# ipastore/glue-factory-colon

Measured on AMD Instinct MI355X. Metric: image-pairs/sec (SuperPoint+LightGlue, 1024 kpts, 640x480), higher is better.
Workload: dtype f32; 1 GPU; SuperPoint-open + LightGlue, 1024 kpts, 640x480 synthetic pairs (BASELINE.json configs[1]); keypoints=1024, parallelism=dp1 (pairs sharded, one final gather), weights=name-seeded seed 0 (no network), pairs_gathered=32, rccl_ranks=1

## Files before the change

### glue-factory-colon_amd/csrc/gemm.hip

```cpp
#include <stdlib.h>

#include "common.h"

#define GBK 32

struct GemmArgs {
  const float* A0;
  const float* A1;
  const float* W;
  const float* bias;
  const float* scale;
  const float* shift;
  const float* residual;
  const float* rot_cos;
  const float* rot_sin;
  const float* rot_cs;
  float* Y;
  long long strideA, strideW, strideY;
  int lda0, lda1, ldw, ldy;
  int K0, K1, M, N, rot_cols;
  float alpha;
  int xcd_remap;
#if defined(GEMM_DIAG) && (GEMM_DIAG & 16)
  unsigned long long* stamps;
#endif
};
#if defined(GEMM_DIAG) && (GEMM_DIAG & 16)
static unsigned long long* g_diag_stamps = nullptr;
extern "C" void gfc_diag_set_gemm_stamps(void* p) { g_diag_stamps = (unsigned long long*)p; }
#define GEMM_STAMP(i_)                                                                               \
  do {                                                                                               \
    if (g.stamps && lane == 0) stamp_base[i_] = __builtin_readcyclecounter();                        \
  } while (0)
#else
#define GEMM_STAMP(i_) do {} while (0)
#endif

template <int MODE, int NS, int RPS, int ELD>
__device__ __forceinline__ void gemm_epilogue_round_fast(const GemmArgs& g, const float* patch, float* Y, int row0, int er,
                                                         int ec, int colb, int rd, float4 bi4, float4 sc4, float4 sh4) {
  float4 opa = make_float4(0.f, 0.f, 0.f, 0.f), opb = opa;
  const float* pa = nullptr;
  const float* pb = nullptr;
  size_t pstep = (size_t)RPS * 64;
  if constexpr (MODE == 1) {
    pa = g.rot_cos + (size_t)row0 * 64 + rd;
    pb = g.rot_sin + (size_t)row0 * 64 + rd;
    opa = *reinterpret_cast<const float4*>(pa);
    opb = *reinterpret_cast<const float4*>(pb);
  } else if constexpr (MODE == 2) {
    pa = g.residual + (size_t)row0 * g.ldy + colb;
    pstep = (size_t)RPS * g.ldy;
    opa = *reinterpret_cast<const float4*>(pa);
  } else if constexpr (MODE == 3) {
    pa = g.rot_cs + (size_t)row0 * 64 + rd;
    opa = *reinterpret_cast<const float4*>(pa);
  }
  float* yp = Y + (size_t)row0 * g.ldy + colb;
  const size_t ystep = (size_t)RPS * g.ldy;
#pragma unroll
  for (int i = 0; i < NS; ++i) {
    float4 na = opa, nb = opb;
    if (i + 1 < NS) {
      if constexpr (MODE != 0) {
        pa += pstep;
        na = *reinterpret_cast<const float4*>(pa);
      }
      if constexpr (MODE == 1) {
        pb += pstep;
        nb = *reinterpret_cast<const float4*>(pb);
      }
    }
    float4 v = *reinterpret_cast<const float4*>(patch + (er + RPS * i) * ELD + ec);
    v.x += bi4.x; v.y += bi4.y; v.z += bi4.z; v.w += bi4.w;
    if constexpr (MODE == 1) {
      const float x = v.x, y = v.y, zz = v.z, w = v.w;
      v.x = x * opa.x + (-y) * opb.x;
      v.y = y * opa.y + x * opb.y;
      v.z = zz * opa.z + (-w) * opb.z;
      v.w = w * opa.w + zz * opb.w;
    }
    if constexpr (MODE == 3) {
      const float x = v.x, y = v.y, zz = v.z, w = v.w;
      v.x = x * opa.x + (-y) * opa.y;
      v.y = y * opa.x + x * opa.y;
      v.z = zz * opa.z + (-w) * opa.w;
      v.w = w * opa.z + zz * opa.w;
    }
    v.x = v.x * sc4.x + sh4.x; v.y = v.y * sc4.y + sh4.y; v.z = v.z * sc4.z + sh4.z; v.w = v.w * sc4.w + sh4.w;
    v.x *= g.alpha; v.y *= g.alpha; v.z *= g.alpha; v.w *= g.alpha;
    if constexpr (MODE == 2) { v.x = opa.x + v.x; v.y = opa.y + v.y; v.z = opa.z + v.z; v.w = opa.w + v.w; }
    *reinterpret_cast<float4*>(yp) = v;
    yp += ystep;
    opa = na; opb = nb;
  }
}

template <int NW, int MT, int MTN = MT>
__device__ __forceinline__ void gemm_epilogue(const GemmArgs& g, f32x16 (&acc)[MT][MTN], float* smem, float* Y, int m0,
                                              int n0, int wm, int wn, int lane, int wave) {
  constexpr int WT = 32 * MTN;
  constexpr int WTM = 32 * MT;
  const int l31 = lane & 31, h = lane >> 5;
  if (((g.rot_cos == nullptr && g.rot_cs == nullptr) || n0 >= g.rot_cols) && g.residual == nullptr) {
#pragma unroll
    for (int nt = 0; nt < MTN; ++nt) {
      const int col = n0 + wn * WT + nt * 32 + l31;
      const bool col_ok = col < g.N;
      const int cc = col_ok ? col : g.N - 1;
      float bi = g.bias ? g.bias[cc] : 0.f;
      float sc = g.scale ? g.scale[cc] : 1.f;
      float sh = g.shift ? g.shift[cc] : 0.f;
      asm volatile("" : "+v"(bi), "+v"(sc), "+v"(sh));
      const bool full = m0 + wm * WTM + MT * 32 <= g.M && n0 + wn * WT + MTN * 32 <= g.N;
#pragma unroll
      for (int mt = 0; mt < MT; ++mt) {
        const int row0 = m0 + wm * WTM + mt * 32;
        if (full) {
          float* yp = Y + (size_t)(row0 + 4 * h) * g.ldy + col;
#pragma unroll
          for (int r = 0; r < 16; ++r) {
            const float v = ((acc[mt][nt][r] + bi) * sc + sh) * g.alpha;
            yp[(size_t)((r & 3) + 8 * (r >> 2)) * g.ldy] = v;
          }
        } else {
#pragma unroll
          for (int r = 0; r < 16; ++r) {
            const int row = row0 + acc_row(r, h);
            const float v = ((acc[mt][nt][r] + bi) * sc + sh) * g.alpha;
            if (row < g.M && col_ok) Y[(size_t)row * g.ldy + col] = v;
          }
        }
      }
    }
    return;
  }
  constexpr int ELD = WT + 4;
  constexpr int LPR = WT / 4;
  constexpr int RPS = 64 / LPR;
  float* patch = smem + wave * 32 * ELD;
  const bool vec_ok = (g.ldy % 4 == 0) && ((reinterpret_cast<size_t>(Y) & 15) == 0) &&
                      (!g.residual || (reinterpret_cast<size_t>(g.residual) & 15) == 0);
  const int er = lane / LPR, ec = (lane % LPR) * 4;
  const int colb = n0 + wn * WT + ec;
  float4 bi4 = make_float4(0.f, 0.f, 0.f, 0.f), sc4 = make_float4(1.f, 1.f, 1.f, 1.f), sh4 = bi4;
  {
    float* bp4 = reinterpret_cast<float*>(&bi4);
    float* sp4 = reinterpret_cast<float*>(&sc4);
    float* hp4 = reinterpret_cast<float*>(&sh4);
#pragma unroll
    for (int j = 0; j < 4; ++j) {
      const int cc = min(colb + j, g.N - 1);
      if (g.bias) bp4[j] = g.bias[cc];
      if (g.scale) { sp4[j] = g.scale[cc]; hp4[j] = g.shift[cc]; }
    }
  }
  const bool rot = (g.rot_cos != nullptr || g.rot_cs != nullptr) && colb < g.rot_cols;
  const int rd = colb & 63;
  asm volatile("" : "+v"(bi4.x), "+v"(bi4.y), "+v"(bi4.z), "+v"(bi4.w));
  asm volatile("" : "+v"(sc4.x), "+v"(sc4.y), "+v"(sc4.z), "+v"(sc4.w));
  asm volatile("" : "+v"(sh4.x), "+v"(sh4.y), "+v"(sh4.z), "+v"(sh4.w));
  const bool rot_w = (g.rot_cos != nullptr || g.rot_cs != nullptr) && n0 + wn * WT < g.rot_cols;
  const bool fast = vec_ok && m0 + wm * WTM + MT * 32 <= g.M && n0 + wn * WT + WT <= g.N && !(rot_w && g.residual);
#pragma unroll
  for (int mt = 0; mt < MT; ++mt) {
    if (fast) {
      constexpr int NS = 32 / RPS;
      const int row0 = m0 + wm * WTM + mt * 32 + er;
      __builtin_amdgcn_fence(__ATOMIC_RELEASE, "wavefront");
      __builtin_amdgcn_wave_barrier();
#pragma unroll
      for (int nt = 0; nt < MTN; ++nt)
#pragma unroll
        for (int r = 0; r < 16; ++r) patch[acc_row(r, h) * ELD + nt * 32 + l31] = acc[mt][nt][r];
      __builtin_amdgcn_fence(__ATOMIC_ACQ_REL, "wavefront");
      __builtin_amdgcn_wave_barrier();
      if (rot_w && g.rot_cs) gemm_epilogue_round_fast<3, NS, RPS, ELD>(g, patch, Y, row0, er, ec, colb, rd, bi4, sc4, sh4);
      else if (rot_w) gemm_epilogue_round_fast<1, NS, RPS, ELD>(g, patch, Y, row0, er, ec, colb, rd, bi4, sc4, sh4);
      else if (g.residual) gemm_epilogue_round_fast<2, NS, RPS, ELD>(g, patch, Y, row0, er, ec, colb, rd, bi4, sc4, sh4);
      else gemm_epilogue_round_fast<0, NS, RPS, ELD>(g, patch, Y, row0, er, ec, colb, rd, bi4, sc4, sh4);
      continue;
    }
    __builtin_amdgcn_fence(__ATOMIC_RELEASE, "wavefront");
    __builtin_amdgcn_wave_barrier();
#pragma unroll
    for (int nt = 0; nt < MTN; ++nt)
#pragma unroll
      for (int r = 0; r < 16; ++r) patch[acc_row(r, h) * ELD + nt * 32 + l31] = acc[mt][nt][r];
    __builtin_amdgcn_fence(__ATOMIC_ACQ_REL, "wavefront");
    __builtin_amdgcn_wave_barrier();
#pragma unroll
    for (int i = 0; i < 32 / RPS; ++i) {
      const int lr = er + RPS * i;
      const int row = m0 + wm * WTM + mt * 32 + lr;
      float4 v = *reinterpret_cast<const float4*>(patch + lr * ELD + ec);
      if (row >= g.M) continue;
      v.x += bi4.x; v.y += bi4.y; v.z += bi4.z; v.w += bi4.w;
      if (rot) {
        float4 c, sn;
        if (g.rot_cs) {
          const float4 cs = *reinterpret_cast<const float4*>(g.rot_cs + (size_t)row * 64 + rd);
          c = make_float4(cs.x, cs.x, cs.z, cs.z);
          sn = make_float4(cs.y, cs.y, cs.w, cs.w);
        } else {
          c = *reinterpret_cast<const float4*>(g.rot_cos + (size_t)row * 64 + rd);
          sn = *reinterpret_cast<const float4*>(g.rot_sin + (size_t)row * 64 + rd);
        }
        const float x = v.x, y = v.y, zz = v.z, w = v.w;
        v.x = x * c.x + (-y) * sn.x;
        v.y = y * c.y + x * sn.y;
        v.z = zz * c.z + (-w) * sn.z;
        v.w = w * c.w + zz * sn.w;
      }
      v.x = v.x * sc4.x + sh4.x; v.y = v.y * sc4.y + sh4.y; v.z = v.z * sc4.z + sh4.z; v.w = v.w * sc4.w + sh4.w;
      v.x *= g.alpha; v.y *= g.alpha; v.z *= g.alpha; v.w *= g.alpha;
      const size_t o = (size_t)row * g.ldy + colb;
      if (vec_ok && colb + 3 < g.N) {
        if (g.residual) {
          const float4 rs = *reinterpret_cast<const float4*>(g.residual + o);
          v.x = rs.x + v.x; v.y = rs.y + v.y; v.z = rs.z + v.z; v.w = rs.w + v.w;
        }
        *reinterpret_cast<float4*>(Y + o) = v;
      } else {
        const float* vp = reinterpret_cast<const float*>(&v);
#pragma unroll
        for (int j = 0; j < 4; ++j)
          if (colb + j < g.N) Y[o + j] = g.residual ? g.residual[o + j] + vp[j] : vp[j];
      }
    }
  }
}

template <int NW, int MT, int BK, int MTN = MT>
__global__ __launch_bounds__(128 * NW, MT * MTN > 4 ? 2 : (BK == 16 ? 4 : 2)) void gemm_nt_kernel(GemmArgs g) {
  constexpr int T = 128 * NW;
  constexpr int GBM = 64 * MT;
  constexpr int BN = 32 * MTN * NW;
  constexpr int GLD = BK + 4;
  constexpr int C4 = BK / 4;
  constexpr int RPP = T / C4;
  constexpr int NA = GBM / RPP;
  constexpr int NB = BN / RPP;
  constexpr int TILE = (GBM + BN) * GLD;
  extern __shared__ __attribute__((aligned(16))) float smem[];

  const int tid = threadIdx.x;
  const int lane = tid & 63, wave = tid >> 6;
  const int l31 = lane & 31, h = lane >> 5;
  const int wm = wave / NW, wn = wave % NW;
  unsigned bx = blockIdx.x, by = blockIdx.y, bz = blockIdx.z;
  if (g.xcd_remap) {
    const unsigned per_z = gridDim.x * gridDim.y;
    unsigned t = gfc_xcd_chunk(bx + gridDim.x * (by + gridDim.y * bz), per_z * gridDim.z);
    bz = t / per_z;
    t -= bz * per_z;
    by = t / gridDim.x;
    bx = t - by * gridDim.x;
  }
  const int m0 = by * GBM, n0 = bx * BN;
  const long long z = bz;
  const float* A0 = g.A0 + z * g.strideA;
  const float* A1 = g.A1 ? g.A1 + z * g.strideA : nullptr;
  const float* W = g.W + z * g.strideW;
  float* Y = g.Y + z * g.strideY;
  const int ktiles = (g.K0 + g.K1) / BK;
#if defined(GEMM_DIAG) && (GEMM_DIAG & 16)
  unsigned long long* stamp_base =
      g.stamps ? g.stamps + ((size_t)(blockIdx.x + gridDim.x * (blockIdx.y + gridDim.y * blockIdx.z)) * (T / 64) + wave) * 8
               : nullptr;
  if (g.stamps && lane == 0) {
    unsigned hw, xcc;
    asm volatile("s_getreg_b32 %0, hwreg(HW_REG_HW_ID)" : "=s"(hw));
    asm volatile("s_getreg_b32 %0, hwreg(HW_REG_XCC_ID)" : "=s"(xcc));
    stamp_base[5] = hw;
    stamp_base[6] = xcc;
  }
  GEMM_STAMP(0);
#endif

  const int s_c4 = (tid % C4) * 4;
  const int q_ = tid / C4;
  const int s_r0 = C4 == 4 ? ((q_ & ~7) | ((q_ & 1) << 2) | ((q_ >> 1) & 3)) : q_;
  const int ar0 = min(m0 + s_r0, g.M - 1), ar1 = min(m0 + s_r0 + RPP, g.M - 1);
  const int ar2 = min(m0 + s_r0 + 2 * RPP, g.M - 1), ar3 = min(m0 + s_r0 + 3 * RPP, g.M - 1);
  const float* w0p = W + (size_t)min(n0 + s_r0, g.N - 1) * g.ldw + s_c4;
  const float* w1p = W + (size_t)min(n0 + s_r0 + RPP, g.N - 1) * g.ldw + s_c4;
  const float* w2p = W + (size_t)min(n0 + s_r0 + 2 * RPP, g.N - 1) * g.ldw + s_c4;
  const float* w3p = W + (size_t)min(n0 + s_r0 + 3 * RPP, g.N - 1) * g.ldw + s_c4;
  static_assert((NB == 1 || NB == 2 || NB == 4) && (NA == 1 || NA == 2 || NA == 4), "staging layout");
  float4 areg0, areg1, areg2, areg3, wreg0, wreg1, wreg2, wreg3;
  areg1 = wreg1 = areg2 = areg3 = wreg2 = wreg3 = make_float4(0.f, 0.f, 0.f, 0.f);
#define GEMM_LOAD_TILE(kt)                                                                           \
  do {                                                                                               \
    const int k0_ = (kt) * BK;                                                                       \
    const bool first_ = k0_ < g.K0;                                                                  \
    const float* ab_ = (first_ ? A0 : A1) + (first_ ? k0_ : k0_ - g.K0) + s_c4;                      \
    const size_t ld_ = first_ ? g.lda0 : g.lda1;                                                     \
    areg0 = *reinterpret_cast<const float4*>(ab_ + ar0 * ld_);                                       \
    if constexpr (NA >= 2) areg1 = *reinterpret_cast<const float4*>(ab_ + ar1 * ld_);                \
    if constexpr (NA == 4) {                                                                         \
      areg2 = *reinterpret_cast<const float4*>(ab_ + ar2 * ld_);                                     \
      areg3 = *reinterpret_cast<const float4*>(ab_ + ar3 * ld_);                                     \
    }                                                                                                \
    wreg0 = *reinterpret_cast<const float4*>(w0p + k0_);                                             \
    if constexpr (NB >= 2) wreg1 = *reinterpret_cast<const float4*>(w1p + k0_);                      \
    if constexpr (NB == 4) {                                                                         \
      wreg2 = *reinterpret_cast<const float4*>(w2p + k0_);                                           \
      wreg3 = *reinterpret_cast<const float4*>(w3p + k0_);                                           \
    }                                                                                                \
  } while (0)
#define GEMM_STORE_TILE(buf_)                                                                        \
  do {                                                                                               \
    float* as_ = smem + (buf_) * TILE + s_r0 * GLD + s_c4;                                           \
    float* bs_ = as_ + GBM * GLD;                                                                    \
    *reinterpret_cast<float4*>(as_) = areg0;                                                         \
    if constexpr (NA >= 2) *reinterpret_cast<float4*>(as_ + RPP * GLD) = areg1;                      \
    if constexpr (NA == 4) {                                                                         \
      *reinterpret_cast<float4*>(as_ + 2 * RPP * GLD) = areg2;                                       \
      *reinterpret_cast<float4*>(as_ + 3 * RPP * GLD) = areg3;                                       \
    }                                                                                                \
    *reinterpret_cast<float4*>(bs_) = wreg0;                                                         \
    if constexpr (NB >= 2) *reinterpret_cast<float4*>(bs_ + RPP * GLD) = wreg1;                      \
    if constexpr (NB == 4) {                                                                         \
      *reinterpret_cast<float4*>(bs_ + 2 * RPP * GLD) = wreg2;                                       \
      *reinterpret_cast<float4*>(bs_ + 3 * RPP * GLD) = wreg3;                                       \
    }                                                                                                \
  } while (0)

  f32x16 acc[MT][MTN];
#pragma unroll
  for (int mt = 0; mt < MT; ++mt)
#pragma unroll
    for (int nt = 0; nt < MTN; ++nt)
#pragma unroll
      for (int r = 0; r < 16; ++r) acc[mt][nt][r] = 0.f;

  const int a_off = (wm * 32 * MT + l31) * GLD + 4 * h;
  const int b_off = GBM * GLD + (wn * 32 * MTN + l31) * GLD + 4 * h;

  GEMM_LOAD_TILE(0);
  GEMM_STORE_TILE(0);
  if (ktiles > 1) GEMM_LOAD_TILE(1);
  __syncthreads();
  GEMM_STAMP(1);
  for (int kt = 0; kt < ktiles; ++kt) {
    if (kt + 1 < ktiles) {
      GEMM_STORE_TILE((kt + 1) & 1);
      if (kt + 2 < ktiles) GEMM_LOAD_TILE(kt + 2);
    }
    const float* ap = smem + (kt & 1) * TILE + a_off;
    const float* bp = smem + (kt & 1) * TILE + b_off;
#pragma unroll
    for (int gk = 0; gk < BK / 8; ++gk) {
      float4 af[MT], bf[MTN];
#pragma unroll
      for (int mt = 0; mt < MT; ++mt) af[mt] = *reinterpret_cast<const float4*>(ap + mt * 32 * GLD + 8 * gk);
#pragma unroll
      for (int nt = 0; nt < MTN; ++nt) bf[nt] = *reinterpret_cast<const float4*>(bp + nt * 32 * GLD + 8 * gk);
#pragma unroll
      for (int mt = 0; mt < MT; ++mt)
#pragma unroll
        for (int nt = 0; nt < MTN; ++nt) {
          acc[mt][nt] = mfma32(af[mt].x, bf[nt].x, acc[mt][nt]);
          acc[mt][nt] = mfma32(af[mt].y, bf[nt].y, acc[mt][nt]);
          acc[mt][nt] = mfma32(af[mt].z, bf[nt].z, acc[mt][nt]);
          acc[mt][nt] = mfma32(af[mt].w, bf[nt].w, acc[mt][nt]);
        }
    }
    __syncthreads();
  }
  GEMM_STAMP(2);

  gemm_epilogue<NW, MT, MTN>(g, acc, smem, Y, m0, n0, wm, wn, lane, wave);
#if defined(GEMM_DIAG) && (GEMM_DIAG & 16)
  GEMM_STAMP(3);
  asm volatile("s_waitcnt vmcnt(0)" ::: "memory");
  GEMM_STAMP(4);
#endif
}

#define GW_BN 512

__device__ __forceinline__ float halfwave_transpose_sum32(const float (&x)[32], int l31) {
  float y16[16], y8[8], y4[4], y2[2];
  const bool b0 = l31 & 1, b1 = l31 & 2, b2 = l31 & 4, b3 = l31 & 8, b4 = l31 & 16;
#pragma unroll
  for (int i = 0; i < 16; ++i) {
    const float mine = b0 ? x[16 + i] : x[i], theirs = b0 ? x[i] : x[16 + i];
    y16[i] = mine + __shfl_xor(theirs, 1);
  }
#pragma unroll
  for (int i = 0; i < 8; ++i) {
    const float mine = b1 ? y16[8 + i] : y16[i], theirs = b1 ? y16[i] : y16[8 + i];
    y8[i] = mine + __shfl_xor(theirs, 2);
  }
#pragma unroll
  for (int i = 0; i < 4; ++i) {
    const float mine = b2 ? y8[4 + i] : y8[i], theirs = b2 ? y8[i] : y8[4 + i];
    y4[i] = mine + __shfl_xor(theirs, 4);
  }
#pragma unroll
  for (int i = 0; i < 2; ++i) {
    const float mine = b3 ? y4[2 + i] : y4[i], theirs = b3 ? y4[i] : y4[2 + i];
    y2[i] = mine + __shfl_xor(theirs, 8);
  }
  const float mine = b4 ? y2[1] : y2[0], theirs = b4 ? y2[0] : y2[1];
  return mine + __shfl_xor(theirs, 16);
}

#define FF_HLD 148
template <bool MLP>
__global__ __launch_bounds__(512, 2) void gemm_rows512_ln_gelu_kernel(GemmArgs g, const float* __restrict__ gamma,
                                                                      const float* __restrict__ beta,
                                                                      const float* __restrict__ W3, int ldw3,
                                                                      const float* __restrict__ b3) {
  constexpr int BM = 128, BK = 16, LD = BK + 4, C4 = BK / 4;
  constexpr int TILE = (BM + GW_BN) * LD;
  extern __shared__ __attribute__((aligned(16))) float smem[];
  const int tid = threadIdx.x, lane = tid & 63, wave = tid >> 6;
  const int l31 = lane & 31, h = lane >> 5;
  const int wm = wave >> 2, wn = wave & 3;
  const int m0 = blockIdx.x * BM;
  const float* A0 = g.A0;
  const float* A1 = g.A1;
  const int ktiles = (g.K0 + g.K1) / BK;
#if defined(GEMM_DIAG) && (GEMM_DIAG & 16)
  unsigned long long* stamp_base = g.stamps ? g.stamps + ((size_t)blockIdx.x * 8 + wave) * 8 : nullptr;
  if (g.stamps && lane == 0) {
    unsigned hw, xcc;
    asm volatile("s_getreg_b32 %0, hwreg(HW_REG_HW_ID)" : "=s"(hw));
    asm volatile("s_getreg_b32 %0, hwreg(HW_REG_XCC_ID)" : "=s"(xcc));
    stamp_base[5] = hw;
    stamp_base[6] = xcc;
  }
  GEMM_STAMP(0);
#endif

  const int s_c4 = (tid % C4) * 4;
  const int q_ = tid / C4;
  const int s_r0 = (q_ & ~7) | ((q_ & 1) << 2) | ((q_ >> 1) & 3);
  const size_t ar = (size_t)min(m0 + s_r0, g.M - 1);
  const float* w0p = g.W + (size_t)(s_r0)*g.ldw + s_c4;
  const float* w1p = w0p + (size_t)128 * g.ldw;
  const float* w2p = w0p + (size_t)256 * g.ldw;
  const float* w3p = w0p + (size_t)384 * g.ldw;
  float4 areg = make_float4(0.f, 0.f, 0.f, 0.f), wreg0, wreg1, wreg2, wreg3;
#define GW_LOAD(kt)                                                              \
  do {                                                                           \
    const int k0_ = (kt) * BK;                                                   \
    const bool first_ = k0_ < g.K0;                                              \
    const float* ab_ = (first_ ? A0 : A1) + (first_ ? k0_ : k0_ - g.K0) + s_c4;  \
    const size_t ld_ = first_ ? g.lda0 : g.lda1;                                 \
    areg = *reinterpret_cast<const float4*>(ab_ + ar * ld_);                     \
    wreg0 = *reinterpret_cast<const float4*>(w0p + k0_);                         \
    wreg1 = *reinterpret_cast<const float4*>(w1p + k0_);                         \
    wreg2 = *reinterpret_cast<const float4*>(w2p + k0_);                         \
    wreg3 = *reinterpret_cast<const float4*>(w3p + k0_);                         \
  } while (0)
#define GW_STORE(buf_)                                                           \
  do {                                                                           \
    float* bs_ = smem + (buf_) * TILE + BM * LD + s_r0 * LD + s_c4;              \
    *reinterpret_cast<float4*>(smem + (buf_) * TILE + s_r0 * LD + s_c4) = areg;  \
    *reinterpret_cast<float4*>(bs_) = wreg0;                                     \
    *reinterpret_cast<float4*>(bs_ + 128 * LD) = wreg1;                          \
    *reinterpret_cast<float4*>(bs_ + 256 * LD) = wreg2;                          \
    *reinterpret_cast<float4*>(bs_ + 384 * LD) = wreg3;                          \
  } while (0)

  f32x16 acc[2][4];
#pragma unroll
  for (int mt = 0; mt < 2; ++mt)
#pragma unroll
    for (int nt = 0; nt < 4; ++nt)
#pragma unroll
      for (int r = 0; r < 16; ++r) acc[mt][nt][r] = 0.f;

  const int a_off = (wm * 64 + l31) * LD + 4 * h;
  const int b_off = BM * LD + (wn * 128 + l31) * LD + 4 * h;

  GW_LOAD(0);
  GW_STORE(0);
  if (ktiles > 1) GW_LOAD(1);
  __syncthreads();
  GEMM_STAMP(1);
  for (int kt = 0; kt < ktiles; ++kt) {
    if (kt + 1 < ktiles) {
      GW_STORE((kt + 1) & 1);
      if (kt + 2 < ktiles) GW_LOAD(kt + 2);
    }
    const float* ap = smem + (kt & 1) * TILE + a_off;
    const float* bp = smem + (kt & 1) * TILE + b_off;
#pragma unroll
    for (int gk = 0; gk < BK / 8; ++gk) {
      float4 af[2], bf[4];
#pragma unroll
      for (int mt = 0; mt < 2; ++mt) af[mt] = *reinterpret_cast<const float4*>(ap + mt * 32 * LD + 8 * gk);
#pragma unroll
      for (int nt = 0; nt < 4; ++nt) bf[nt] = *reinterpret_cast<const float4*>(bp + nt * 32 * LD + 8 * gk);
#pragma unroll
      for (int mt = 0; mt < 2; ++mt)
#pragma unroll
        for (int nt = 0; nt < 4; ++nt) {
          acc[mt][nt] = mfma32(af[mt].x, bf[nt].x, acc[mt][nt]);
          acc[mt][nt] = mfma32(af[mt].y, bf[nt].y, acc[mt][nt]);
          acc[mt][nt] = mfma32(af[mt].z, bf[nt].z, acc[mt][nt]);
          acc[mt][nt] = mfma32(af[mt].w, bf[nt].w, acc[mt][nt]);
        }
    }
    __syncthreads();
  }
#undef GW_LOAD
#undef GW_STORE
  GEMM_STAMP(2);
  constexpr int W3T = 256 * LD;
  float* const Hs = smem;
  float* const Ws = smem + 128 * FF_HLD;
  const float* w3p0 = MLP ? W3 + (size_t)s_r0 * ldw3 + s_c4 : nullptr;
  const float* w3p1 = MLP ? w3p0 + (size_t)128 * ldw3 : nullptr;
#define FF_LOAD(T_)                                                   \
  do {                                                                \
    wreg0 = *reinterpret_cast<const float4*>(w3p0 + (T_) * 16);       \
    wreg1 = *reinterpret_cast<const float4*>(w3p1 + (T_) * 16);       \
  } while (0)
#define FF_STORE(buf_)                                                \
  do {                                                                \
    float* bs_ = Ws + (buf_) * W3T + s_r0 * LD + s_c4;                \
    *reinterpret_cast<float4*>(bs_) = wreg0;                          \
    *reinterpret_cast<float4*>(bs_ + 128 * LD) = wreg1;               \
  } while (0)
  if constexpr (MLP) FF_LOAD(0);

  float* red = smem;
  float* stat = smem + 4 * BM;
  float bi[4], ga[4], be[4];
#pragma unroll
  for (int nt = 0; nt < 4; ++nt) {
    const int col = wn * 128 + nt * 32 + l31;
    bi[nt] = g.bias ? g.bias[col] : 0.f;
    ga[nt] = gamma[col];
    be[nt] = beta[col];
  }
#pragma unroll
  for (int nt = 0; nt < 4; ++nt) asm volatile("" : "+v"(bi[nt]), "+v"(ga[nt]), "+v"(be[nt]));
#pragma unroll
  for (int mt = 0; mt < 2; ++mt)
#pragma unroll
    for (int nt = 0; nt < 4; ++nt)
#pragma unroll
      for (int r = 0; r < 16; ++r) acc[mt][nt][r] += bi[nt];
  const int vb = ((l31 & 1) << 4) | ((l31 & 2) << 2) | (l31 & 4) | ((l31 & 8) >> 2) | ((l31 & 16) >> 4);
  const int my_row = wm * 64 + (vb >> 4) * 32 + acc_row(vb & 15, h);
  float mu[2][16];
  {
    float x[32];
#pragma unroll
    for (int mt = 0; mt < 2; ++mt)
#pragma unroll
      for (int r = 0; r < 16; ++r)
        x[mt * 16 + r] = (acc[mt][0][r] + acc[mt][1][r]) + (acc[mt][2][r] + acc[mt][3][r]);
    red[wn * BM + my_row] = halfwave_transpose_sum32(x, l31);
  }
  __syncthreads();
  if (tid < BM) stat[tid] = ((red[tid] + red[BM + tid]) + (red[2 * BM + tid] + red[3 * BM + tid])) * (1.f / 512.f);
  __syncthreads();
#pragma unroll
  for (int mt = 0; mt < 2; ++mt)
#pragma unroll
    for (int gq = 0; gq < 4; ++gq) {
      const float4 m4 = *reinterpret_cast<const float4*>(stat + wm * 64 + mt * 32 + 8 * gq + 4 * h);
      mu[mt][4 * gq] = m4.x; mu[mt][4 * gq + 1] = m4.y; mu[mt][4 * gq + 2] = m4.z; mu[mt][4 * gq + 3] = m4.w;
    }
  {
    float x[32];
#pragma unroll
    for (int mt = 0; mt < 2; ++mt)
#pragma unroll
      for (int r = 0; r < 16; ++r) {
        const float d0 = acc[mt][0][r] - mu[mt][r], d1 = acc[mt][1][r] - mu[mt][r];
        const float d2 = acc[mt][2][r] - mu[mt][r], d3 = acc[mt][3][r] - mu[mt][r];
        x[mt * 16 + r] = (d0 * d0 + d1 * d1) + (d2 * d2 + d3 * d3);
      }
    red[wn * BM + my_row] = halfwave_transpose_sum32(x, l31);
  }
  __syncthreads();
  if (tid < BM) {
    const float var = ((red[tid] + red[BM + tid]) + (red[2 * BM + tid] + red[3 * BM + tid])) * (1.f / 512.f);
    stat[BM + tid] = 1.f / sqrtf(var + 1e-5f);
  }
  __syncthreads();
  if constexpr (!MLP) GEMM_STAMP(3);
  const bool full_rows = m0 + BM <= g.M;
#pragma unroll
  for (int mt = 0; mt < 2; ++mt) {
#pragma unroll
    for (int gq = 0; gq < 4; ++gq) {
      const float4 r4 = *reinterpret_cast<const float4*>(stat + BM + wm * 64 + mt * 32 + 8 * gq + 4 * h);
      const float rs[4] = {r4.x, r4.y, r4.z, r4.w};
#pragma unroll
      for (int j = 0; j < 4; ++j) {
        const int r = 4 * gq + j;
        const int row = m0 + wm * 64 + mt * 32 + acc_row(r, h);
        if constexpr (MLP) {
#pragma unroll
          for (int nt = 0; nt < 4; ++nt)
            acc[mt][nt][r] = gfc_gelu((acc[mt][nt][r] - mu[mt][r]) * rs[j] * ga[nt] + be[nt]);
        } else if (full_rows || row < g.M) {
          float* yp = g.Y + (size_t)row * g.ldy + wn * 128 + l31;
#pragma unroll
          for (int nt = 0; nt < 4; ++nt) {
            yp[nt * 32] = gfc_gelu((acc[mt][nt][r] - mu[mt][r]) * rs[j] * ga[nt] + be[nt]);
          }
        }
      }
    }
  }
#if defined(GEMM_DIAG) && (GEMM_DIAG & 16)
  if constexpr (MLP) GEMM_STAMP(3);
  else GEMM_STAMP(4);
#endif
  if constexpr (MLP) {
    f32x16 acc2[2][2];
#pragma unroll
    for (int mt = 0; mt < 2; ++mt)
#pragma unroll
      for (int nt = 0; nt < 2; ++nt)
#pragma unroll
        for (int r = 0; r < 16; ++r) acc2[mt][nt][r] = 0.f;
    const int a_off3 = (wm * 64 + l31) * FF_HLD + 4 * h;
    const int b_off3 = (wn * 64 + l31) * LD + 4 * h;
    FF_STORE(0);
    FF_LOAD(1);
    __syncthreads();
#pragma unroll 1
    for (int c = 0; c < 4; ++c) {
      if (wn == c) {
#pragma unroll
        for (int mt = 0; mt < 2; ++mt)
#pragma unroll
          for (int nt = 0; nt < 4; ++nt)
#pragma unroll
            for (int r = 0; r < 16; ++r)
              Hs[(wm * 64 + mt * 32 + acc_row(r, h)) * FF_HLD + nt * 32 + l31] = acc[mt][nt][r];
      }
      __syncthreads();
#pragma unroll 1
      for (int t = 0; t < 8; ++t) {
        const int T = c * 8 + t;
        if (T + 1 < 32) {
          FF_STORE((T + 1) & 1);
          if (T + 2 < 32) FF_LOAD(T + 2);
        }
        const float* ap = Hs + a_off3 + 16 * t;
        const float* bp = Ws + (T & 1) * W3T + b_off3;
#pragma unroll
        for (int gk = 0; gk < 2; ++gk) {
          float4 af[2], bf[2];
#pragma unroll
          for (int mt = 0; mt < 2; ++mt) af[mt] = *reinterpret_cast<const float4*>(ap + mt * 32 * FF_HLD + 8 * gk);
#pragma unroll
          for (int nt = 0; nt < 2; ++nt) bf[nt] = *reinterpret_cast<const float4*>(bp + nt * 32 * LD + 8 * gk);
#pragma unroll
          for (int mt = 0; mt < 2; ++mt)
#pragma unroll
            for (int nt = 0; nt < 2; ++nt) {
              acc2[mt][nt] = mfma32(af[mt].x, bf[nt].x, acc2[mt][nt]);
              acc2[mt][nt] = mfma32(af[mt].y, bf[nt].y, acc2[mt][nt]);
              acc2[mt][nt] = mfma32(af[mt].z, bf[nt].z, acc2[mt][nt]);
              acc2[mt][nt] = mfma32(af[mt].w, bf[nt].w, acc2[mt][nt]);
            }
        }
        __syncthreads();
      }
    }
    GEMM_STAMP(4);
#pragma unroll
    for (int nt = 0; nt < 2; ++nt) {
      const int col = wn * 64 + nt * 32 + l31;
      float bi3 = b3 ? b3[col] : 0.f;
      asm volatile("" : "+v"(bi3));
#pragma unroll
      for (int mt = 0; mt < 2; ++mt) {
        const int row0 = m0 + wm * 64 + mt * 32 + 4 * h;
        const size_t o0 = (size_t)row0 * g.ldy + col;
        float rv[16];
        if (full_rows) {
#pragma unroll
          for (int r = 0; r < 16; ++r) rv[r] = g.residual ? g.residual[o0 + (size_t)((r & 3) + 8 * (r >> 2)) * g.ldy] : 0.f;
#pragma unroll
          for (int r = 0; r < 16; ++r) g.Y[o0 + (size_t)((r & 3) + 8 * (r >> 2)) * g.ldy] = rv[r] + (acc2[mt][nt][r] + bi3);
        } else {
#pragma unroll
          for (int r = 0; r < 16; ++r) {
            const int row = row0 + (r & 3) + 8 * (r >> 2);
            if (row < g.M) {
              const size_t o = (size_t)row * g.ldy + col;
              g.Y[o] = (g.residual ? g.residual[o] : 0.f) + (acc2[mt][nt][r] + bi3);
            }
          }
        }
      }
    }
    GEMM_STAMP(7);
  }
#undef FF_LOAD
#undef FF_STORE
}

extern "C" int gfc_ffn_fused(const float* A0, int lda0, int K0, const float* A1, int lda1, int K1, const float* W0,
                             int ldw0, const float* b0, const float* gamma, const float* beta, const float* W3, int ldw3,
                             const float* b3, const float* residual, float* Y, int ldy, int M, void* stream) {
  if (!A0 || !W0 || !gamma || !beta || !W3 || !Y || M <= 0 || K0 <= 0 || K0 % GBK || K1 % GBK || K1 < 0)
    return GFC_ERR_INVALID;
  if ((K1 > 0) != (A1 != nullptr)) return GFC_ERR_INVALID;
  if (lda0 % 4 || (A1 && lda1 % 4) || ldw0 % 4 || ldw3 % 4 || ldw3 < GW_BN || ldy < 256) return GFC_ERR_INVALID;
  GemmArgs g = {};
  g.A0 = A0; g.A1 = A1; g.W = W0; g.bias = b0; g.residual = residual; g.Y = Y;
  g.lda0 = lda0; g.lda1 = lda1; g.ldw = ldw0; g.ldy = ldy;
  g.K0 = K0; g.K1 = K1; g.M = M; g.N = GW_BN; g.alpha = 1.f;
  constexpr size_t k1 = (size_t)2 * (128 + GW_BN) * 20, k2 = (size_t)128 * FF_HLD + (size_t)2 * 256 * 20;
  constexpr size_t lds = (k1 > k2 ? k1 : k2) * sizeof(float);
  static std::atomic<unsigned long long> lds_ok{0};
  gfc_allow_dynamic_lds((const void*)gemm_rows512_ln_gelu_kernel<true>, lds, lds_ok);
#if defined(GEMM_DIAG) && (GEMM_DIAG & 16)
  g.stamps = g_diag_stamps;
#endif
  hipLaunchKernelGGL(gemm_rows512_ln_gelu_kernel<true>, dim3((M + 127) / 128), dim3(512), lds, (hipStream_t)stream, g,
                     gamma, beta, W3, ldw3, b3);
  GFC_LAUNCH_CHECK();
  return GFC_OK;
}

extern "C" int gfc_linear_layernorm_gelu(const float* A0, int lda0, int K0, const float* A1, int lda1, int K1,
                                         const float* W, int ldw, const float* bias, const float* gamma,
                                         const float* beta, float* Y, int ldy, int M, int N, void* stream) {
  if (!A0 || !W || !gamma || !beta || !Y || M <= 0 || K0 <= 0 || K0 % GBK || K1 % GBK || K1 < 0) return GFC_ERR_INVALID;
  if ((K1 > 0) != (A1 != nullptr)) return GFC_ERR_INVALID;
  if (lda0 % 4 || (A1 && lda1 % 4) || ldw % 4 || ldy < N) return GFC_ERR_INVALID;
  if (N != GW_BN) return GFC_ERR_UNSUPPORTED;
  GemmArgs g = {};
  g.A0 = A0; g.A1 = A1; g.W = W; g.bias = bias; g.Y = Y;
  g.lda0 = lda0; g.lda1 = lda1; g.ldw = ldw; g.ldy = ldy;
  g.K0 = K0; g.K1 = K1; g.M = M; g.N = N; g.alpha = 1.f;
  constexpr size_t lds = (size_t)2 * (128 + GW_BN) * 20 * sizeof(float);
  static std::atomic<unsigned long long> lds_ok{0};
  gfc_allow_dynamic_lds((const void*)gemm_rows512_ln_gelu_kernel<false>, lds, lds_ok);
#if defined(GEMM_DIAG) && (GEMM_DIAG & 16)
  g.stamps = g_diag_stamps;
#endif
  hipLaunchKernelGGL(gemm_rows512_ln_gelu_kernel<false>, dim3((M + 127) / 128), dim3(512), lds, (hipStream_t)stream, g,
                     gamma, beta, (const float*)nullptr, 0, (const float*)nullptr);
  GFC_LAUNCH_CHECK();
  return GFC_OK;
}

template <int NW, int MT, int BK, int MTN = MT>
static int launch_gemm_t(const GemmArgs& g, int batch, hipStream_t st) {
  constexpr int BM = 64 * MT, BN = 32 * MTN * NW;
  constexpr size_t kloop = (size_t)2 * (BM + BN) * (BK + 4), patches = (size_t)2 * NW * 32 * (32 * MTN + 4);
  const size_t lds = (kloop > patches ? kloop : patches) * sizeof(float);
  static std::atomic<unsigned long long> lds_ok{0};
  if (lds > 64 * 1024) gfc_allow_dynamic_lds((const void*)gemm_nt_kernel<NW, MT, BK, MTN>, lds, lds_ok);
  dim3 grid((g.N + BN - 1) / BN, (g.M + BM - 1) / BM, batch);
  GemmArgs ga = g;
  ga.xcd_remap = (long long)grid.x * grid.y * grid.z >= 16;
#if defined(GEMM_DIAG) && (GEMM_DIAG & 16)
  ga.stamps = g_diag_stamps;
#endif
  hipLaunchKernelGGL((gemm_nt_kernel<NW, MT, BK, MTN>), grid, dim3(128 * NW), lds, st, ga);
  GFC_LAUNCH_CHECK();
  return GFC_OK;
}

static int launch_gemm(const GemmArgs& g, int batch, hipStream_t st) {
  const int forced = gfc_knobs().gemm_tile;
  auto tiles = [&](int bm, int bn) { return (long long)((g.M + bm - 1) / bm) * ((g.N + bn - 1) / bn) * batch; };
  int choice = (forced == 3 || forced == 4) ? forced : 0;
  if (!choice) {
    choice = tiles(128, 128) >= 768 ? 4 : 3;
  }
  if (choice == 4) return launch_gemm_t<2, 2, 16>(g, batch, st);
  return launch_gemm_t<2, 1, 32>(g, batch, st);
}

extern "C" int gfc_linear(const float* A0, int lda0, int K0, const float* A1, int lda1, int K1, const float* W, int ldw,
                          const float* bias, const float* scale, const float* shift, float alpha,
                          const float* residual, const float* rot_cos, const float* rot_sin, int rot_cols, float* Y,
                          int ldy, int M, int N, void* stream) {
  if (!A0 || !W || !Y || M <= 0 || N <= 0 || K0 <= 0 || K0 % GBK || K1 % GBK || K1 < 0) return GFC_ERR_INVALID;
  if ((K1 > 0) != (A1 != nullptr)) return GFC_ERR_INVALID;
  if ((scale == nullptr) != (shift == nullptr)) return GFC_ERR_INVALID;
  if ((rot_cos == nullptr) != (rot_sin == nullptr)) return GFC_ERR_INVALID;
  if (rot_cos && (rot_cols % 64 != 0)) return GFC_ERR_INVALID;
  if (lda0 % 4 || (A1 && lda1 % 4) || ldw % 4) return GFC_ERR_INVALID;
  GemmArgs g = {};
  g.A0 = A0; g.A1 = A1; g.W = W; g.bias = bias; g.scale = scale; g.shift = shift; g.residual = residual;
  g.rot_cos = rot_cos; g.rot_sin = rot_sin; g.Y = Y;
  g.strideA = g.strideW = g.strideY = 0;
  g.lda0 = lda0; g.lda1 = lda1; g.ldw = ldw; g.ldy = ldy;
  g.K0 = K0; g.K1 = K1; g.M = M; g.N = N; g.rot_cols = rot_cols; g.alpha = alpha;
  return launch_gemm(g, 1, (hipStream_t)stream);
}

int gfc_linear_rot_packed(const float* A0, int lda0, int K0, const float* W, int ldw, const float* bias, const float* rot_cs,
                          int rot_cols, float* Y, int ldy, int M, int N, void* stream) {
  if (!A0 || !W || !Y || !rot_cs || M <= 0 || N <= 0 || K0 <= 0 || K0 % GBK || rot_cols % 64 || lda0 % 4 || ldw % 4)
    return GFC_ERR_INVALID;
  GemmArgs g = {};
  g.A0 = A0; g.W = W; g.bias = bias; g.rot_cs = rot_cs; g.Y = Y;
  g.lda0 = lda0; g.ldw = ldw; g.ldy = ldy;
  g.K0 = K0; g.K1 = 0; g.M = M; g.N = N; g.rot_cols = rot_cols; g.alpha = 1.f;
  return launch_gemm(g, 1, (hipStream_t)stream);
}

extern "C" int gfc_batched_nt(const float* A, int lda, long long strideA, const float* Bm, int ldb, long long strideB,
                              float* Y, int ldy, long long strideY, int M, int N, int K, int batch, void* stream) {
  if (!A || !Bm || !Y || M <= 0 || N <= 0 || K <= 0 || K % GBK || batch <= 0) return GFC_ERR_INVALID;
  if (lda % 4 || ldb % 4 || strideA % 4 || strideB % 4) return GFC_ERR_INVALID;
  GemmArgs g = {};
  g.A0 = A; g.A1 = nullptr; g.W = Bm; g.bias = nullptr; g.scale = nullptr; g.shift = nullptr; g.residual = nullptr;
  g.rot_cos = nullptr; g.rot_sin = nullptr; g.Y = Y;
  g.strideA = strideA; g.strideW = strideB; g.strideY = strideY;
  g.lda0 = lda; g.lda1 = 0; g.ldw = ldb; g.ldy = ldy;
  g.K0 = K; g.K1 = 0; g.M = M; g.N = N; g.rot_cols = 0; g.alpha = 1.f;
  return launch_gemm(g, batch, (hipStream_t)stream);
}
```

Before: 931.7 image-pairs/sec.

## Stream FFN weight tiles into LDS via global_load_lds DMA with XOR swizzle

```diff
diff --git a/glue-factory-colon_amd/csrc/gemm.hip b/glue-factory-colon_amd/csrc/gemm.hip
--- a/glue-factory-colon_amd/csrc/gemm.hip
+++ b/glue-factory-colon_amd/csrc/gemm.hip
@@ -380,6 +380,7 @@
 }
 
 #define GW_BN 512
+typedef __attribute__((address_space(3))) void* lds_ptr_t;
 
 __device__ __forceinline__ float halfwave_transpose_sum32(const float (&x)[32], int l31) {
   float y16[16], y8[8], y4[4], y2[2];
@@ -415,7 +416,8 @@
                                                                       const float* __restrict__ W3, int ldw3,
                                                                       const float* __restrict__ b3) {
   constexpr int BM = 128, BK = 16, LD = BK + 4, C4 = BK / 4;
-  constexpr int TILE = (BM + GW_BN) * LD;
+  constexpr int WT0 = GW_BN * BK;
+  constexpr int A_OFF = 2 * WT0, ATILE = BM * LD;
   extern __shared__ __attribute__((aligned(16))) float smem[];
   const int tid = threadIdx.x, lane = tid & 63, wave = tid >> 6;
   const int l31 = lane & 31, h = lane >> 5;
@@ -440,11 +442,7 @@
   const int q_ = tid / C4;
   const int s_r0 = (q_ & ~7) | ((q_ & 1) << 2) | ((q_ >> 1) & 3);
   const size_t ar = (size_t)min(m0 + s_r0, g.M - 1);
-  const float* w0p = g.W + (size_t)(s_r0)*g.ldw + s_c4;
-  const float* w1p = w0p + (size_t)128 * g.ldw;
-  const float* w2p = w0p + (size_t)256 * g.ldw;
-  const float* w3p = w0p + (size_t)384 * g.ldw;
-  float4 areg = make_float4(0.f, 0.f, 0.f, 0.f), wreg0, wreg1, wreg2, wreg3;
+  float4 areg = make_float4(0.f, 0.f, 0.f, 0.f);
 #define GW_LOAD(kt)                                                              \
   do {                                                                           \
     const int k0_ = (kt) * BK;                                                   \
@@ -452,19 +450,30 @@
     const float* ab_ = (first_ ? A0 : A1) + (first_ ? k0_ : k0_ - g.K0) + s_c4;  \
     const size_t ld_ = first_ ? g.lda0 : g.lda1;                                 \
     areg = *reinterpret_cast<const float4*>(ab_ + ar * ld_);                     \
-    wreg0 = *reinterpret_cast<const float4*>(w0p + k0_);                         \
-    wreg1 = *reinterpret_cast<const float4*>(w1p + k0_);                         \
-    wreg2 = *reinterpret_cast<const float4*>(w2p + k0_);                         \
-    wreg3 = *reinterpret_cast<const float4*>(w3p + k0_);                         \
   } while (0)
-#define GW_STORE(buf_)                                                           \
+#define GW_STORE(buf_) *reinterpret_cast<float4*>(smem + A_OFF + (buf_) * ATILE + s_r0 * LD + s_c4) = areg
+  const int d_rl = lane >> 2, d_c = 4 * ((lane & 3) ^ ((d_rl >> 2) & 3));
+  const float* wsrc = g.W + (size_t)(64 * wave + d_rl) * g.ldw + d_c;
+  const size_t wstep = (size_t)16 * g.ldw;
+  const unsigned smem_lds = (unsigned)(size_t)(lds_ptr_t)smem;
+#define FF_GLDS(gsrc_, foff_)  \
+  do {                                                                                                              \
+    unsigned keep_;                                                                                                 \
+    const unsigned la_ = smem_lds + 4u * (unsigned)(foff_);                                                         \
+    asm volatile("s_mov_b32 %0, m0\n\ts_mov_b32 m0, %2\n\ts_nop 0\n\tglobal_load_lds_dwordx4 %1, off\n\ts_mov_b32 m0, %0" \
+                 : "=&s"(keep_)                                                                                     \
+                 : "v"(gsrc_), "s"(__builtin_amdgcn_readfirstlane(la_))                                             \
+                 : "memory");                                                                                       \
+  } while (0)
+#define FF_DMA_WAIT() asm volatile("s_waitcnt vmcnt(0)" ::: "memory")
+#define GW_DMA(kt, buf_)                                                         \
   do {                                                                           \
-    float* bs_ = smem + (buf_) * TILE + BM * LD + s_r0 * LD + s_c4;              \
-    *reinterpret_cast<float4*>(smem + (buf_) * TILE + s_r0 * LD + s_c4) = areg;  \
-    *reinterpret_cast<float4*>(bs_) = wreg0;                                     \
-    *reinterpret_cast<float4*>(bs_ + 128 * LD) = wreg1;                          \
-    *reinterpret_cast<float4*>(bs_ + 256 * LD) = wreg2;                          \
-    *reinterpret_cast<float4*>(bs_ + 384 * LD) = wreg3;                          \
+    const float* s_ = wsrc + (kt) * BK;                                          \
+    const int d_ = (buf_) * WT0 + 1024 * wave;                                   \
+    FF_GLDS(s_, d_);                                                             \
+    FF_GLDS(s_ + wstep, d_ + 256);                                               \
+    FF_GLDS(s_ + 2 * wstep, d_ + 512);                                           \
+    FF_GLDS(s_ + 3 * wstep, d_ + 768);                                           \
   } while (0)
 
   f32x16 acc[2][4];
@@ -475,28 +484,34 @@
 #pragma unroll
       for (int r = 0; r < 16; ++r) acc[mt][nt][r] = 0.f;
 
-  const int a_off = (wm * 64 + l31) * LD + 4 * h;
-  const int b_off = BM * LD + (wn * 128 + l31) * LD + 4 * h;
-
+  const int a_off = A_OFF + (wm * 64 + l31) * LD + 4 * h;
+  const int sw = (l31 >> 2) & 3;
+  const int wch0 = 4 * (h ^ sw), wch1 = 4 * ((2 + h) ^ sw);
+  const int b_off = (wn * 128 + l31) * BK;
+
+  GW_DMA(0, 0);
   GW_LOAD(0);
   GW_STORE(0);
+  FF_DMA_WAIT();
+  __builtin_amdgcn_sched_barrier(0);
   if (ktiles > 1) GW_LOAD(1);
   __syncthreads();
   GEMM_STAMP(1);
   for (int kt = 0; kt < ktiles; ++kt) {
     if (kt + 1 < ktiles) {
       GW_STORE((kt + 1) & 1);
+      GW_DMA(kt + 1, (kt + 1) & 1);
       if (kt + 2 < ktiles) GW_LOAD(kt + 2);
     }
-    const float* ap = smem + (kt & 1) * TILE + a_off;
-    const float* bp = smem + (kt & 1) * TILE + b_off;
+    const float* ap = smem + (kt & 1) * ATILE + a_off;
+    const float* bp = smem + (kt & 1) * WT0 + b_off;
 #pragma unroll
     for (int gk = 0; gk < BK / 8; ++gk) {
       float4 af[2], bf[4];
 #pragma unroll
       for (int mt = 0; mt < 2; ++mt) af[mt] = *reinterpret_cast<const float4*>(ap + mt * 32 * LD + 8 * gk);
 #pragma unroll
-      for (int nt = 0; nt < 4; ++nt) bf[nt] = *reinterpret_cast<const float4*>(bp + nt * 32 * LD + 8 * gk);
+      for (int nt = 0; nt < 4; ++nt) bf[nt] = *reinterpret_cast<const float4*>(bp + nt * 32 * BK + (gk ? wch1 : wch0));
 #pragma unroll
       for (int mt = 0; mt < 2; ++mt)
 #pragma unroll
@@ -507,31 +522,30 @@
           acc[mt][nt] = mfma32(af[mt].w, bf[nt].w, acc[mt][nt]);
         }
     }
+    __builtin_amdgcn_sched_barrier(0);
+    FF_DMA_WAIT();
     __syncthreads();
   }
 #undef GW_LOAD
 #undef GW_STORE
+#undef GW_DMA
   GEMM_STAMP(2);
-  constexpr int W3T = 256 * LD;
-  float* const Hs = smem;
-  float* const Ws = smem + 128 * FF_HLD;
-  const float* w3p0 = MLP ? W3 + (size_t)s_r0 * ldw3 + s_c4 : nullptr;
-  const float* w3p1 = MLP ? w3p0 + (size_t)128 * ldw3 : nullptr;
-#define FF_LOAD(T_)                                                   \
+  constexpr int W3T = 256 * BK;
+  float* const Ws = smem;
+  float* const Hs = smem + 2 * W3T;
+  const float* w3src = MLP ? W3 + (size_t)(32 * wave + d_rl) * ldw3 + d_c : nullptr;
+  const size_t w3step = (size_t)16 * ldw3;
+#define FF_DMA(T_, buf_)                                              \
   do {                                                                \
-    wreg0 = *reinterpret_cast<const float4*>(w3p0 + (T_) * 16);       \
-    wreg1 = *reinterpret_cast<const float4*>(w3p1 + (T_) * 16);       \
+    const float* s_ = w3src + (T_) * 16;                              \
+    const int d_ = (buf_) * W3T + 512 * wave;          \
+    FF_GLDS(s_, d_);                                                  \
+    FF_GLDS(s_ + w3step, d_ + 256);                                   \
   } while (0)
-#define FF_STORE(buf_)                                                \
-  do {                                                                \
-    float* bs_ = Ws + (buf_) * W3T + s_r0 * LD + s_c4;                \
-    *reinterpret_cast<float4*>(bs_) = wreg0;                          \
-    *reinterpret_cast<float4*>(bs_ + 128 * LD) = wreg1;               \
-  } while (0)
-  if constexpr (MLP) FF_LOAD(0);
-
-  float* red = smem;
-  float* stat = smem + 4 * BM;
+  if constexpr (MLP) FF_DMA(0, 0);
+
+  float* red = smem + 2 * W3T;
+  float* stat = red + 4 * BM;
   float bi[4], ga[4], be[4];
 #pragma unroll
   for (int nt = 0; nt < 4; ++nt) {
@@ -627,9 +641,8 @@
 #pragma unroll
         for (int r = 0; r < 16; ++r) acc2[mt][nt][r] = 0.f;
     const int a_off3 = (wm * 64 + l31) * FF_HLD + 4 * h;
-    const int b_off3 = (wn * 64 + l31) * LD + 4 * h;
-    FF_STORE(0);
-    FF_LOAD(1);
+    const int b_off3 = (wn * 64 + l31) * BK;
+    FF_DMA_WAIT();
     __syncthreads();
 #pragma unroll 1
     for (int c = 0; c < 4; ++c) {
@@ -646,10 +659,7 @@
 #pragma unroll 1
       for (int t = 0; t < 8; ++t) {
         const int T = c * 8 + t;
-        if (T + 1 < 32) {
-          FF_STORE((T + 1) & 1);
-          if (T + 2 < 32) FF_LOAD(T + 2);
-        }
+        if (T + 1 < 32) FF_DMA(T + 1, (T + 1) & 1);
         const float* ap = Hs + a_off3 + 16 * t;
         const float* bp = Ws + (T & 1) * W3T + b_off3;
 #pragma unroll
@@ -658,7 +668,7 @@
 #pragma unroll
           for (int mt = 0; mt < 2; ++mt) af[mt] = *reinterpret_cast<const float4*>(ap + mt * 32 * FF_HLD + 8 * gk);
 #pragma unroll
-          for (int nt = 0; nt < 2; ++nt) bf[nt] = *reinterpret_cast<const float4*>(bp + nt * 32 * LD + 8 * gk);
+          for (int nt = 0; nt < 2; ++nt) bf[nt] = *reinterpret_cast<const float4*>(bp + nt * 32 * BK + (gk ? wch1 : wch0));
 #pragma unroll
           for (int mt = 0; mt < 2; ++mt)
 #pragma unroll
@@ -669,6 +679,8 @@
               acc2[mt][nt] = mfma32(af[mt].w, bf[nt].w, acc2[mt][nt]);
             }
         }
+        __builtin_amdgcn_sched_barrier(0);
+        FF_DMA_WAIT();
         __syncthreads();
       }
     }
@@ -702,8 +714,9 @@
     }
     GEMM_STAMP(7);
   }
-#undef FF_LOAD
-#undef FF_STORE
+#undef FF_DMA
+#undef FF_DMA_WAIT
+#undef FF_GLDS
 }
 
 extern "C" int gfc_ffn_fused(const float* A0, int lda0, int K0, const float* A1, int lda1, int K1, const float* W0,
@@ -717,7 +730,7 @@
   g.A0 = A0; g.A1 = A1; g.W = W0; g.bias = b0; g.residual = residual; g.Y = Y;
   g.lda0 = lda0; g.lda1 = lda1; g.ldw = ldw0; g.ldy = ldy;
   g.K0 = K0; g.K1 = K1; g.M = M; g.N = GW_BN; g.alpha = 1.f;
-  constexpr size_t k1 = (size_t)2 * (128 + GW_BN) * 20, k2 = (size_t)128 * FF_HLD + (size_t)2 * 256 * 20;
+  constexpr size_t k1 = (size_t)2 * (GW_BN * 16 + 128 * 20), k2 = (size_t)2 * 256 * 16 + (size_t)128 * FF_HLD;
   constexpr size_t lds = (k1 > k2 ? k1 : k2) * sizeof(float);
   static std::atomic<unsigned long long> lds_ok{0};
   gfc_allow_dynamic_lds((const void*)gemm_rows512_ln_gelu_kernel<true>, lds, lds_ok);
@@ -741,7 +754,7 @@
   g.A0 = A0; g.A1 = A1; g.W = W; g.bias = bias; g.Y = Y;
   g.lda0 = lda0; g.lda1 = lda1; g.ldw = ldw; g.ldy = ldy;
   g.K0 = K0; g.K1 = K1; g.M = M; g.N = N; g.alpha = 1.f;
-  constexpr size_t lds = (size_t)2 * (128 + GW_BN) * 20 * sizeof(float);
+  constexpr size_t lds = (size_t)2 * (GW_BN * 16 + 128 * 20) * sizeof(float);
   static std::atomic<unsigned long long> lds_ok{0};
   gfc_allow_dynamic_lds((const void*)gemm_rows512_ln_gelu_kernel<false>, lds, lds_ok);
 #if defined(GEMM_DIAG) && (GEMM_DIAG & 16)
```

Measured after the change: 937.2 image-pairs/sec (median of 6 runs). No clear change (+0.6%).
